# si220/Forest-SLAM

Hardware: AMD Instinct MI355X
Metric: stereo frames/sec (extract+match+local-BA) at 600p, 1/8 MI355X; ATE RMSE (higher is better)
Workload: dtype mixed: u8/u16 integer (FAST, BRIEF, Hamming, SGM), f32 (ORB angle/Harris, back-projection), f64 (PnP, BA incl. its Schur GEMM on f64 MFMA)

## Files before the change

### forest-slam_amd/csrc/fvo_internal.h

```cpp
#pragma once

#include <hip/hip_runtime.h>

#include <cmath>
#include <cstdint>
#include <string>
#include <vector>

#include "../../include/fvo.h"

#define FVO_MAX_LEVELS 12

struct OrbGeom {
  int nlevels;
  int w[FVO_MAX_LEVELS], h[FVO_MAX_LEVELS];
  float scale[FVO_MAX_LEVELS];
  int64_t off[FVO_MAX_LEVELS + 1];
  int row0[FVO_MAX_LEVELS + 1];
  int nfeat[FVO_MAX_LEVELS];
  int64_t cand_off[FVO_MAX_LEVELS + 1];
  int64_t total_px;
  int total_rows;
  int64_t cand_total;
  bool angle_pass;
};

struct ResizeTab {
  int32_t* xofs;
  int32_t* xc1;
  int32_t* yofs;
  int32_t* yc1;
  int64_t xoff[FVO_MAX_LEVELS], yoff[FVO_MAX_LEVELS];
};

constexpr int kBaMaxWindow = 21;
constexpr int kEmMaxCap = 5040;
constexpr int kRansacMaxIters = 1000;

#define FVO_KERNELS(X)                                                                                    \
  X(KN_ORB_COPY, "orb_copy_level0") X(KN_ORB_RESIZE, "orb_resize") X(KN_ORB_FAST, "orb_fast_score")       \
  X(KN_ORB_NMS_COUNT, "orb_nms_count") X(KN_ORB_ROW_SCAN, "orb_row_scan") X(KN_ORB_COMPACT, "orb_nms_compact") \
  X(KN_ORB_SELECT1, "orb_select_fast") X(KN_ORB_HARRIS, "orb_harris") X(KN_ORB_SELECT2, "orb_select_harris") \
  X(KN_ORB_OFFSETS, "orb_offsets") X(KN_ORB_ANGLE, "orb_angle") X(KN_ORB_BLUR, "orb_blur")                \
  X(KN_ORB_BRIEF, "orb_brief") X(KN_BF_ARGMIN, "bf_argmin") X(KN_BF_FINISH, "bf_finish")                  \
  X(KN_SG_VERT, "sgbm_vert") X(KN_SG_ROWS, "sgbm_rows") X(KN_SG_MEDIAN, "sgbm_median")                    \
  X(KN_BACKPROJECT, "backproject") X(KN_PNP, "pnp_ransac") X(KN_BA_STEREO, "ba_stereo")                   \
  X(KN_BA_BUILD, "ba_build") X(KN_BA_SOLVE, "ba_solve") X(KN_GATHER, "gather_matches")                    \
  X(KN_ESSENTIAL, "essential_ransac") X(KN_RECOVER, "recover_pose") X(KN_INGEST, "ingest_undistort_gray") \
  X(KN_MOTION_BLUR, "motion_blur") X(KN_MAP_XFORM, "map_transform") X(KN_VOXEL, "voxel_down_sample")      \
  X(KN_BF_KNN, "bf_knn") X(KN_BF_RATIO, "bf_ratio") X(KN_SPK_LOCAL, "speckle_local")                      \
  X(KN_SPK_SEAMS, "speckle_seams") X(KN_SPK_SUM, "speckle_sum") X(KN_SPK_APPLY, "speckle_apply")
#define FVO_KERNEL_ID(id, name) id,
enum FvoKernel { FVO_KERNELS(FVO_KERNEL_ID) KN_COUNT };
#undef FVO_KERNEL_ID

struct TimingRec {
  int id;
  hipEvent_t a, b;
};

struct fvo_ctx {
  int device = 0;
  uint64_t tmask = 0;
  std::vector<TimingRec> trecs;
  std::vector<hipEvent_t> tpool;
  fvo_config cfg{};
  OrbGeom g{};
  std::string err;
  int kp_cap = 0;
  int64_t ws_bytes = 0;
  std::vector<void*> allocs;
  uint8_t* pyr = nullptr;
  uint8_t* blur = nullptr;
  int orb_last_batch = 0;
  uint8_t* score = nullptr;
  uint32_t* cand = nullptr;
  uint64_t* hel = nullptr;
  int32_t* ncand = nullptr;
  int32_t* nsel1 = nullptr;
  int32_t* nsel2 = nullptr;
  int32_t* koff = nullptr;
  int32_t* scratch = nullptr;
  int64_t scratch_per = 0;
  ResizeTab rt{};
  int32_t* umax = nullptr;
  uint32_t* bf_rowkey = nullptr;
  uint32_t* bf_colkey = nullptr;
  uint32_t* bf_knn = nullptr;
  uint16_t* sg_V = nullptr;
  uint16_t* sg_M = nullptr;
  uint32_t* sg_ckpt = nullptr;
  int16_t* sg_raw = nullptr;
  uint64_t* sg_hand = nullptr;
  uint32_t* sg_ctl = nullptr;
  struct {
    bool valid = false;
    const void* matches = nullptr;
    const void* nmatch = nullptr;
    const void* stereo = nullptr;
    int nframes = 0, first_end = 0, nwin = 0, first_valid = 0;
  } ba_births;
  double* pnp_hyp = nullptr;
  int32_t* pnp_sub = nullptr;
  int16_t* rs_table = nullptr;
  int32_t rs_table_iters = 0;
  double* pnp_models = nullptr;
  double* pnp_ws = nullptr;
  int32_t* pnp_good = nullptr;
  void* pnp_state = nullptr;
  float* pnp_pts = nullptr;
  int32_t* pnp_plan = nullptr;
  int32_t pnp_max_iters = 0;
  uint8_t* fast_rec = nullptr;
  void* ba_ws = nullptr;
  int64_t ba_win_bytes = 0;
  hipStream_t ba_s2 = nullptr;
  hipEvent_t ba_fork = nullptr, ba_join = nullptr;
  double* em_x = nullptr;
  double* em_models = nullptr;
  int32_t* em_good = nullptr;
  int8_t* em_nmod = nullptr;
  double* em_ws = nullptr;
  void* em_state = nullptr;
  int32_t em_max_iters = 0;
  int32_t rectify_budget = FVO_RECTIFY_LDS_BYTES;
};

int fvo_fail(fvo_ctx* ctx, const std::string& msg);
#define FVO_HIP(ctx, expr)                                                                 \
  do {                                                                                     \
    hipError_t e_ = (expr);                                                                \
    if (e_ != hipSuccess) return fvo_fail(ctx, std::string(#expr) + ": " + hipGetErrorString(e_)); \
  } while (0)
#define FVO_LAUNCH_CHECK(ctx) FVO_HIP(ctx, hipGetLastError())

hipEvent_t fvo_event(fvo_ctx* ctx);
#define FVO_TIMED(ctx, id, s, ...)                               \
  do {                                                           \
    const bool t_ = ((ctx)->tmask >> (id)) & 1ull;               \
    hipEvent_t a_ = nullptr, b_ = nullptr;                       \
    if (t_) {                                                    \
      a_ = fvo_event(ctx);                                       \
      (void)hipEventRecord(a_, s);                               \
    }                                                            \
    __VA_ARGS__;                                                 \
    if (t_) {                                                    \
      b_ = fvo_event(ctx);                                       \
      (void)hipEventRecord(b_, s);                               \
      (ctx)->trecs.push_back(TimingRec{(int)(id), a_, b_});      \
    }                                                            \
  } while (0)

int orb_init(fvo_ctx* ctx);
int orb_run(fvo_ctx* ctx, const uint8_t* images, int batch, int64_t image_stride, int pitch, float* kp, uint8_t* desc,
            int32_t* counts, int cap, hipStream_t s);
int bf_init(fvo_ctx* ctx);
int bf_run(fvo_ctx* ctx, const uint8_t* q, const int32_t* nq, const uint8_t* t, const int32_t* nt, int batch, int cap,
           int32_t* matches, int32_t* nmatch, hipStream_t s);
int bf_knn_run(fvo_ctx* ctx, const uint8_t* q, const int32_t* nq, const uint8_t* t, const int32_t* nt, int batch,
               int cap, int k, int32_t* knn, hipStream_t s);
int bf_ratio_run(fvo_ctx* ctx, const uint8_t* q, const int32_t* nq, const uint8_t* t, const int32_t* nt, int batch,
                 int cap, double ratio, int mutual, int32_t* matches, int32_t* nmatch, hipStream_t s);
int sgbm_init(fvo_ctx* ctx);
int sgbm_run(fvo_ctx* ctx, const uint8_t* L, const uint8_t* R, int batch, int64_t image_stride, int pitch,
             int16_t* disp, int32_t* status, hipStream_t s);
int pose_init(fvo_ctx* ctx);
int ransac_table_init(fvo_ctx* ctx);
int orb_blur_debug(fvo_ctx* ctx);
int orb_score_debug(fvo_ctx* ctx);
int orb_retain_best_run(fvo_ctx* ctx, const float* keys, int n, int keep, int32_t* idx_out, int32_t* n_out,
                         hipStream_t s);
int backproject_run(fvo_ctx* ctx, const int16_t* disp, const float* kp0, const float* kp1, const int32_t* matches,
                    const int32_t* nmatch, int batch, int cap, const double* K, double baseline, float* P3, float* p2,
                    int32_t* npts, hipStream_t s);
int pnp_run(fvo_ctx* ctx, const float* P3, const float* p2, const int32_t* npts, int batch, int cap, const double* K,
            const double* dist, float reproj, double conf, int iters, double* rvec, double* tvec, double* T,
            int32_t* status, uint8_t* inliers, hipStream_t s);

inline bool host_inv3(const double* S, double* t) {
  double d = S[0] * (S[4] * S[8] - S[5] * S[7]) - S[1] * (S[3] * S[8] - S[5] * S[6]) + S[2] * (S[3] * S[7] - S[4] * S[6]);
  if (d == 0.) return false;
  d = 1. / d;
  t[0] = (S[4] * S[8] - S[5] * S[7]) * d;
  t[1] = (S[2] * S[7] - S[1] * S[8]) * d;
  t[2] = (S[1] * S[5] - S[2] * S[4]) * d;
  t[3] = (S[5] * S[6] - S[3] * S[8]) * d;
  t[4] = (S[0] * S[8] - S[2] * S[6]) * d;
  t[5] = (S[2] * S[3] - S[0] * S[5]) * d;
  t[6] = (S[3] * S[7] - S[4] * S[6]) * d;
  t[7] = (S[1] * S[6] - S[0] * S[7]) * d;
  t[8] = (S[0] * S[4] - S[1] * S[3]) * d;
  return true;
}
inline bool host_all_finite(const double* v, int n) {
  for (int i = 0; i < n; ++i)
    if (!std::isfinite(v[i])) return false;
  return true;
}
inline bool host_ray_w_ok(double w) { return w > 0.0 && std::isfinite(1. / w); }

inline int ingest_stripe_rows(int W, int H) {
  const int s = 4096 / (W > 1 ? W : 1);
  return s < 1 ? 1 : (s > H ? H : s);
}
int ingest_run(fvo_ctx* ctx, const uint8_t* bgr, int batch, int64_t sstride, int spitch, const double* K,
               const double* dist, uint8_t* gray, int64_t dstride, int dpitch, hipStream_t s);
int motion_blur_run(fvo_ctx* ctx, const uint8_t* img, int batch, int64_t sstride, int spitch, int ksize,
                    const int32_t* centers, const int32_t* ncent, int cap, uint8_t* mask, uint8_t* out,
                    int64_t dstride, int dpitch, hipStream_t s);
int map_transform_run(fvo_ctx* ctx, const float* pts, int stride, const int32_t* npts, int batch, int64_t cap,
                      const double* T, int32_t* count, int64_t map_cap, double* out64, float* out32, hipStream_t s);
int chain_poses_run(fvo_ctx* ctx, const double* T, const int32_t* status, const int32_t* npts, int n_seq, int n,
                    double* cum, double* cum_out, int32_t* npts_out, hipStream_t s);
struct FvoRegions {
  fvo_region r[FVO_MAX_REGIONS];
};
int copy_regions_run(fvo_ctx* ctx, int count, const fvo_region* regions, hipStream_t s);
int count_guard_run(fvo_ctx* ctx, const int32_t* cnt, const int32_t* q_cnt, int n, int sets, int32_t* status,
                    int32_t code, int32_t* nkp_out, hipStream_t s);
int64_t voxel_workspace_bytes(int64_t n);
int voxel_run(fvo_ctx* ctx, const double* pts, int64_t n, double voxel, void* ws, double* out,
              int32_t* n_out, int32_t* status, hipStream_t s);
int speckle_run(fvo_ctx* ctx, int16_t* disp, int batch, int H, int W, int64_t image_stride, int pitch, int new_val,
                int max_speckle_size, int max_diff, void* ws, hipStream_t s);
constexpr int kDenseBlock = 1024;
inline int64_t dense_frame_samples(int H, int W, int step) {
  return (int64_t)((H - 1) / step + 1) * ((W - 1) / step + 1);
}
inline int64_t dense_frame_blocks(int H, int W, int step) {
  return (dense_frame_samples(H, W, step) + kDenseBlock - 1) / kDenseBlock;
}
int dense_append_run(fvo_ctx* ctx, const int16_t* disp, int batch, int H, int W, int64_t image_stride, int pitch,
                     const double* K, double baseline, int step, int min_disp16, float z_min, float z_max,
                     const int32_t* frame_keep, const double* T, int32_t* count, int64_t map_cap, double* out64,
                     float* out32, int32_t* n_added, void* ws, hipStream_t s);
int reproject_run(fvo_ctx* ctx, const void* disp, int is_f32, int batch, int H, int W, int64_t image_stride,
                  int pitch, const double* Q, int handle_missing, uint32_t* min_key, float* out, hipStream_t s);
struct RectifyLens {
  double ir[9];
  double fx, fy, u0, v0;
  double k1, k2, p1, p2, k3, k4, k5, k6;
  int rational;
};
int rectify_map_run(fvo_ctx* ctx, const RectifyLens& L, int16_t* map1, uint16_t* map2, hipStream_t s);
int remap_run(fvo_ctx* ctx, const uint8_t* src, int batch, int64_t sstride, int spitch, int channels,
              const int16_t* map1, const uint16_t* map2, uint8_t* dst, int64_t dstride, int dpitch, hipStream_t s);
int rectify_gray_run(fvo_ctx* ctx, const uint8_t* src, int batch, int64_t sstride, int spitch, int channels,
                     const RectifyLens& L, uint8_t* gray, int64_t dstride, int dpitch, hipStream_t s);
constexpr int kSparseMaxLevels = 32;
constexpr int kSparseMaxHalfWindow = 7, kSparseMaxHalfSlide = 8;
struct SparseLevels {
  float scale[kSparseMaxLevels];
  int n;
};
int sparse_stereo_run(fvo_ctx* ctx, const uint8_t* left, const uint8_t* right, int batch, int64_t image_stride,
                      int pitch, const float* kpL, const int32_t* nL, const uint8_t* descL, const float* kpR,
                      const int32_t* nR, const uint8_t* descR, int cap, const fvo_sparse_stereo_params& p,
                      const SparseLevels& levels, const double* K, double baseline, void* ws, float* stereo,
                      int32_t* info, hipStream_t s);
int backproject_stereo_run(fvo_ctx* ctx, const float* stereo, const float* kp1, const int32_t* matches,
// ... 57 lines not shown
```

### forest-slam_amd/csrc/pose.hip

```cpp
#include <cfloat>
#include <cstdlib>
#include <type_traits>

#include "fvo_device.h"
#include "ransac.h"

namespace {

constexpr int kChunk = 64;

constexpr int kBackprojectThreads = 256;

__global__ __launch_bounds__(kBackprojectThreads) void k_backproject(
    const int16_t* __restrict__ disp, const float* __restrict__ kp0, const float* __restrict__ kp1,
    const int32_t* __restrict__ matches, const int32_t* __restrict__ nmatch, int W, int H, int cap, StereoCamF K,
    float* __restrict__ P3, float* __restrict__ p2, int32_t* __restrict__ npts) {
  const int b = blockIdx.x;
  int n = nmatch[b];
  n = n < 0 ? 0 : (n > cap ? cap : n);
  __shared__ int s_w[16];
  __shared__ int s_carry;
  if (threadIdx.x == 0) s_carry = 0;
  __syncthreads();
  for (int base = 0; base < n; base += kBackprojectThreads) {
// ... 1036 lines not shown
  for (int i = lane; i < n; i += 64) {
    const int j = i;
    dundistort(K, (double)p2[2 * j], (double)p2[2 * j + 1], &mn[2 * i]);
    acc[0] += (double)P3[3 * j];
    acc[1] += (double)P3[3 * j + 1];
    acc[2] += (double)P3[3 * j + 2];
  }
#pragma unroll
  for (int k = 0; k < 3; ++k) acc[k] = wave_sum(acc[k]);
  double Mc[3] = {acc[0] / n, acc[1] / n, acc[2] / n};
  double MM[9] = {0, 0, 0, 0, 0, 0, 0, 0, 0};
  for (int i = lane; i < n; i += 64) {
    const int j = i;
    double d[3] = {(double)P3[3 * j] - Mc[0], (double)P3[3 * j + 1] - Mc[1], (double)P3[3 * j + 2] - Mc[2]};
#pragma unroll
    for (int a = 0; a < 3; ++a)
#pragma unroll
      for (int b = 0; b < 3; ++b) MM[a * 3 + b] += d[a] * d[b];
  }
#pragma unroll
  for (int k = 0; k < 9; ++k) MM[k] = wave_sum(MM[k]);
  double W3[3], U3[9], V3[9];
  dsvd<3, 3>(MM, W3, U3, V3);
  const bool planar = W3[2] / W3[1] < 1e-3;
  if (!planar && n < 6) {
    if (lane == 0) sh.flag = 0;
    __syncthreads();
    return;
  }
  double LLp[78];
#pragma unroll
  for (int k = 0; k < 78; ++k) LLp[k] = 0;
  double Rt[9], T[3];
  if (!planar) {
    for (int i = lane; i < n; i += 64) {
      const int j = i;
      double x = -mn[2 * i], y = -mn[2 * i + 1];
      double P[3] = {(double)P3[3 * j], (double)P3[3 * j + 1], (double)P3[3 * j + 2]};
      double r0[12] = {P[0], P[1], P[2], 1., 0, 0, 0, 0, x * P[0], x * P[1], x * P[2], x};
      double r1[12] = {0, 0, 0, 0, P[0], P[1], P[2], 1., y * P[0], y * P[1], y * P[2], y};
      int k = 0;
#pragma unroll
      for (int a = 0; a < 12; ++a)
#pragma unroll
        for (int b = a; b < 12; ++b) LLp[k++] += r0[a] * r0[b] + r1[a] * r1[b];
    }
  } else {
#pragma unroll
    for (int i = 0; i < 3; ++i)
#pragma unroll
      for (int j = 0; j < 3; ++j) Rt[i * 3 + j] = V3[j * 3 + i];
    if (Rt[2] * Rt[2] + Rt[5] * Rt[5] < 1e-10)
#pragma unroll
      for (int i = 0; i < 9; ++i) Rt[i] = (i % 4 == 0);
    if (ddet3(Rt) < 0)
#pragma unroll
      for (int i = 0; i < 9; ++i) Rt[i] = -Rt[i];
#pragma unroll
    for (int i = 0; i < 3; ++i) T[i] = -(Rt[i * 3] * Mc[0] + Rt[i * 3 + 1] * Mc[1] + Rt[i * 3 + 2] * Mc[2]);
    if (lane == 0) {
#pragma unroll
      for (int i = 0; i < 9; ++i) sh.rt[i] = Rt[i];
#pragma unroll
      for (int i = 0; i < 3; ++i) sh.t3[i] = T[i];
    }
    for (int i = lane; i < n; i += 64) {
      const int j = i;
      double s0 = P3[3 * j], s1 = P3[3 * j + 1], s2 = P3[3 * j + 2];
      double X = Rt[0] * s0 + Rt[1] * s1 + Rt[2] * s2 + T[0];
      double Y = Rt[3] * s0 + Rt[4] * s1 + Rt[5] * s2 + T[1];
      double u = mn[2 * i], v = mn[2 * i + 1];
      double r0[9] = {X, Y, 1, 0, 0, 0, -u * X, -u * Y, -u};
      double r1[9] = {0, 0, 0, X, Y, 1, -v * X, -v * Y, -v};
      int k = 0;
#pragma unroll
      for (int a = 0; a < 9; ++a)
#pragma unroll
        for (int b = a; b < 9; ++b) LLp[k++] += r0[a] * r0[b] + r1[a] * r1[b];
    }
  }
#pragma unroll
  for (int k = 0; k < 78; ++k) {
    const double t = wave_sum(LLp[k]);
    if (lane == 0) sh.llp[k] = t;
  }
  __syncthreads();
  if (!planar) dlt12_null(sh.llp, sh.dlt[1], sh.dlt[2], sh.rrt);
  if (lane == 0) dlt_pose(sh, planar);
  __syncthreads();
  double prev[6];
  double lambdaLg10 = -3, prevErrNorm = DBL_MAX;
  int iters = 0;
  for (;;) {
    double e0 = lm_eval(sh, K, P3, p2, n, true);
#pragma unroll
    for (int i = 0; i < 6; ++i) prev[i] = sh.param[i];
    if (lane == 0) {
#pragma unroll
      for (int i = 0; i < 6; ++i) sh.prev[i] = prev[i];
    }
    __syncthreads();
    if (lane == 0) lm_step(sh, lambdaLg10);
    __syncthreads();
    if (iters == 0) prevErrNorm = e0;
    double errNorm;
    for (;;) {
      errNorm = lm_eval(sh, K, P3, p2, n, false);
      if (errNorm > prevErrNorm && ++lambdaLg10 <= 16) {
        if (lane == 0) lm_step(sh, lambdaLg10);
        __syncthreads();
        continue;
      }
      break;
    }
    lambdaLg10 = fmax(lambdaLg10 - 1, -16.0);
    double dn = 0, pn = 0;
#pragma unroll
    for (int i = 0; i < 6; ++i) {
      dn += (sh.param[i] - prev[i]) * (sh.param[i] - prev[i]);
      pn += prev[i] * prev[i];
    }
    double rel = sqrt(dn) / (sqrt(pn) + DBL_EPSILON);
    if (++iters >= 20 || rel < FLT_EPSILON) break;
    prevErrNorm = errNorm;
  }
  if (lane == 0) sh.flag = 1;
  __syncthreads();
}

struct PnpState {
  int maxGood, niters, best_it, n;
};

__global__ void k_pnp_table(int cap, int maxIters, int16_t* __restrict__ table) {
  const int n = blockIdx.x * blockDim.x + threadIdx.x;
  if (n < 6 || n > cap) return;
  fvo_rs::draw_subsets(n, maxIters, table + (int64_t)n * maxIters * 5);
}

__global__ void k_pnp_subsets(const int32_t* __restrict__ npts, int batch, int cap, int maxIters,
                              PnpState* __restrict__ state) {
  const int b = blockIdx.x * blockDim.x + threadIdx.x;
  if (b >= batch) return;
  int n = npts[b];
  n = n < 0 ? 0 : (n > cap ? cap : n);
  PnpState st;
  st.maxGood = 0;
  st.niters = maxIters;
  st.best_it = -1;
  st.n = n;
  state[b] = st;
}

constexpr int PNP_WS = 256;
constexpr int PW_NV = 0, PW_CWS = 48, PW_AL = 60, PW_PWS = 80, PW_US = 95, PW_MTM = 112;

constexpr int PNP_FIRST = 128;
constexpr int PNP_CS = 64, PNP_CA = 8, PNP_CB = 16;

__global__ __launch_bounds__(64) void k_pnp_plan(int batch, int maxIters, const PnpState* __restrict__ state,
                                                 int32_t* __restrict__ plan) {
  const int lane = threadIdx.x;
  int carry[3] = {0, 0, 0};
  const int C[3] = {PNP_CS, PNP_CA, PNP_CB};
  for (int b0 = 0; b0 < batch; b0 += 64) {
    const int b = b0 + lane;
    int rem = 0;
    if (b < batch) {
      const PnpState st = state[b];
      if (st.n >= 6) rem = max(0, min(st.niters, maxIters) - PNP_FIRST);
    }
#pragma unroll
    for (int k = 0; k < 3; ++k) {
      int v = (rem + C[k] - 1) / C[k];
#pragma unroll
      for (int o = 1; o < 64; o <<= 1) {
        const int y = __shfl_up(v, o, 64);
        if (lane >= o) v += y;
      }
      const int incl = v, excl = incl - (rem + C[k] - 1) / C[k];
      if (b < batch) plan[k * (batch + 1) + b] = carry[k] + excl;
      carry[k] += __shfl(incl, 63, 64);
    }
  }
  if (lane < 3) plan[lane * (batch + 1) + batch] = carry[lane];
}

__device__ __forceinline__ void pnp_unit(const int32_t* __restrict__ pre, int batch, int u, int C, int& b, int& base) {
  int lo = 0, hi = batch - 1;
  while (lo < hi) {
    const int mid = (lo + hi + 1) >> 1;
    if (pre[mid] <= u) lo = mid; else hi = mid - 1;
  }
  b = lo;
  base = PNP_FIRST + (u - pre[lo]) * C;
}

template <int C, typename Body>
__device__ __forceinline__ void pnp_units(const int32_t* __restrict__ plan, int k, int batch, int maxIters,
                                          const PnpState* __restrict__ state, Body body) {
  const int32_t* pre = plan ? plan + k * (batch + 1) : nullptr;
  const int total = plan ? pre[batch] : (int)blockIdx.x + 1;
  for (int u = blockIdx.x; u < total; u += gridDim.x) {
    int b, base, lim;
    if (plan) {
      pnp_unit(pre, batch, u, C, b, base);
      lim = maxIters;
    } else {
      b = blockIdx.y;
      base = u * C;
      lim = PNP_FIRST;
    }
    const PnpState st = state[b];
    const int hi = min(min(st.niters, maxIters), lim);
    if (st.n < 6 || base >= hi) continue;
    body(b, base, hi, st.n);
  }
}

__global__ __launch_bounds__(64, 4) void k_pnp_setup(const float* __restrict__ P3all, const float* __restrict__ p2all,
                                                  int cap, Cam K, int maxIters, int batch,
                                                  const int32_t* __restrict__ plan,
                                                  const int16_t* __restrict__ table, int table_iters,
                                                  const PnpState* __restrict__ state, double* __restrict__ ws) {
  extern __shared__ __attribute__((aligned(16))) double smt[];
  double* mt = smt + threadIdx.x;
  pnp_units<PNP_CS>(plan, 0, batch, maxIters, state, [&](int b, int base, int hi, int n) {
    const int it = base + threadIdx.x;
    if (it >= hi) return;
    const float* __restrict__ P3 = P3all + (int64_t)b * cap * 3;
    const float* __restrict__ p2 = p2all + (int64_t)b * cap * 2;
    double* w = ws + ((int64_t)b * maxIters + it) * PNP_WS;
    const int16_t* sb = table + ((int64_t)n * table_iters + it) * 5;
    EPnPd<5> e;
    e.fu = K.fx; e.fv = K.fy; e.uc = K.cx; e.vc = K.cy;
#pragma unroll
    for (int i = 0; i < 5; ++i) {
      int j = sb[i];
#pragma unroll
      for (int c = 0; c < 3; ++c) e.pws[3 * i + c] = (double)P3[j * 3 + c];
      double xy[2];
      dundistort(K, (double)p2[j * 2], (double)p2[j * 2 + 1], xy);
      float fx = (float)xy[0], fy = (float)xy[1];
      e.us[2 * i] = fx * K.fx + K.cx;
      e.us[2 * i + 1] = fy * K.fy + K.cy;
    }
    e.build_mtm<64>(mt);
#pragma unroll 8
    for (int k = 0; k < 144; ++k) w[PW_MTM + k] = mt[k * 64];
#pragma unroll
    for (int r = 0; r < 4; ++r)
#pragma unroll
      for (int k = 0; k < 3; ++k) w[PW_CWS + r * 3 + k] = e.cws[r][k];
#pragma unroll
    for (int k = 0; k < 20; ++k) w[PW_AL + k] = e.alphas[k];
#pragma unroll
    for (int k = 0; k < 15; ++k) w[PW_PWS + k] = e.pws[k];
#pragma unroll
    for (int k = 0; k < 10; ++k) w[PW_US + k] = e.us[k];
  });
}

__global__ __launch_bounds__(64) void k_pnp_hyp_a(int maxIters, int batch, const int32_t* __restrict__ plan,
                                                  const PnpState* __restrict__ state, double* __restrict__ ws) {
  __shared__ double su[8][144];
  const int g = threadIdx.x >> 3, l = threadIdx.x & 7;
  double* u = su[g];
  pnp_units<PNP_CA>(plan, 1, batch, maxIters, state, [&](int b, int base, int hi, int) {
    const int it = base + g;
    if (it >= hi) return;
    double* w = ws + ((int64_t)b * maxIters + it) * PNP_WS;
    for (int k = l; k < 144; k += 8) u[k] = w[PW_MTM + k];
    __builtin_amdgcn_s_waitcnt(0);
    __builtin_amdgcn_wave_barrier();
    jacobi12_null4_group(u, l, w + PW_NV);
  });
}

__global__ __launch_bounds__(64, 3) void k_pnp_hyp_b(const float* __restrict__ P3all, const float* __restrict__ p2all,
                                                  int cap, Cam K, float thr2, int maxIters, int batch,
                                                  const int32_t* __restrict__ plan,
                                                  const PnpState* __restrict__ state, const double* __restrict__ ws,
                                                  double* __restrict__ model, int32_t* __restrict__ good) {
  __shared__ double sL[16][66];
  const int g = threadIdx.x >> 2, l = threadIdx.x & 3;
  double* L = sL[g];
  pnp_units<PNP_CB>(plan, 2, batch, maxIters, state, [&](int b, int base, int hi, int n) {
    const int it = base + g;
    if (it >= hi) return;
    const float* __restrict__ P3 = P3all + (int64_t)b * cap * 3;
    const float* __restrict__ p2 = p2all + (int64_t)b * cap * 2;
    const double* w = ws + ((int64_t)b * maxIters + it) * PNP_WS;
    EPnPd<5, true> e;
    e.fu = K.fx; e.fv = K.fy; e.uc = K.cx; e.vc = K.cy;
    e.pws = w + PW_PWS;
    e.us = w + PW_US;
    e.alphas = w + PW_AL;
    e.cws = reinterpret_cast<const double (*)[3]>(w + PW_CWS);
    const double (*nv)[12] = reinterpret_cast<const double (*)[12]>(w + PW_NV);
    if (l == 0) e.prep(nv, L, L + 60);
    __builtin_amdgcn_s_waitcnt(0);
    __builtin_amdgcn_wave_barrier();
    double R[9], t[3];
    const double err = e.approx(l < 3 ? l + 1 : 3, L, L + 60, nv, R, t);
    const int gb = threadIdx.x & ~3;
    const double e1 = __shfl(err, gb + 1, 64), e2 = __shfl(err, gb + 2, 64);
    int sel = 0;
    double best = __shfl(err, gb, 64);
    if (e1 < best) { best = e1; sel = 1; }
    if (e2 < best) sel = 2;
#pragma unroll
    for (int k = 0; k < 9; ++k) R[k] = __shfl(R[k], gb + sel, 64);
#pragma unroll
    for (int k = 0; k < 3; ++k) t[k] = __shfl(t[k], gb + sel, 64);
    double r[3], dR[27];
    rod_R2r(R, r);
    if (l == 0) {
      double* mo = model + ((int64_t)b * maxIters + it) * 6;
      for (int i = 0; i < 3; ++i) { mo[i] = r[i]; mo[3 + i] = t[i]; }
    }
    rod_r2R(r, R, dR);
    int gcount = 0;
#pragma nounroll
    for (int i = l; i < n; i += 4) {
      double M[3] = {(double)P3[3 * i], (double)P3[3 * i + 1], (double)P3[3 * i + 2]}, uv[2];
      dproject(K, R, dR, t, M, uv, nullptr);
      float du = p2[2 * i] - (float)uv[0], dv = p2[2 * i + 1] - (float)uv[1];
      gcount += (du * du + dv * dv) <= thr2;
    }
    gcount += __shfl_xor(gcount, 1, 4);
    gcount += __shfl_xor(gcount, 2, 4);
    if (l == 0) good[(int64_t)b * maxIters + it] = gcount;
  });
}

__global__ __launch_bounds__(64) void k_pnp_replay(int maxIters, int it_lo, int it_hi, double conf,
                                                   const int32_t* __restrict__ good, PnpState* __restrict__ state) {
  const int b = blockIdx.x, lane = threadIdx.x;
  PnpState st = state[b];
  if (st.n < 6) return;
  for (int base = it_lo; base < it_hi && base < st.niters; base += 64) {
    const int it = base + lane;
    const int g = (it < it_hi && it < st.niters) ? good[(int64_t)b * maxIters + it] : 0;
    for (int j = 0; j < 64; ++j) {
      if (base + j >= it_hi || base + j >= st.niters) break;
      const int gj = __builtin_amdgcn_readlane(g, j);
      if (gj > max(st.maxGood, 4)) {
        st.best_it = base + j;
        st.maxGood = gj;
        st.niters = update_num_iters(conf, (double)(st.n - gj) / st.n, 5, st.niters);
      }
    }
  }
  if (lane == 0) state[b] = st;
}

__global__ __launch_bounds__(64, 2) void k_pnp_refine(const float* __restrict__ P3all, const float* __restrict__ p2all,
                                                   int cap, Cam K, float thr2, int maxIters,
                                                   const PnpState* __restrict__ state,
                                                   const double* __restrict__ model, double* __restrict__ rvec,
                                                   double* __restrict__ tvec, double* __restrict__ T,
                                                   int32_t* __restrict__ status, uint8_t* __restrict__ inliers,
                                                   int32_t* __restrict__ inl_idx, double* __restrict__ mn_buf,
                                                   float* __restrict__ pts) {
  __shared__ PnpShared sh;
  __shared__ float s_pts[5 * kRefineLds];
  const int b = blockIdx.x, lane = threadIdx.x;
  const PnpState st = state[b];
  const int n = st.n;
  const float* P3 = P3all + (int64_t)b * cap * 3;
  const float* p2 = p2all + (int64_t)b * cap * 2;
  double* Tout = T + (int64_t)b * 16;
  if (n < 6 || st.maxGood <= 0) {
    if (lane < 16) Tout[lane] = (lane % 5 == 0) ? 1.0 : 0.0;
    if (lane < 3) { rvec[b * 3 + lane] = 0; tvec[b * 3 + lane] = 0; }
    if (inliers)
      for (int i = lane; i < cap; i += 64) inliers[(int64_t)b * cap + i] = 0;
    if (lane == 0) status[b] = n < 6 ? -1 : 0;
    return;
  }
  const double* mo = model + ((int64_t)b * maxIters + st.best_it) * 6;
  if (lane < 6) sh.best[lane] = mo[lane];
  __syncthreads();
  int* inl = inl_idx + (int64_t)b * cap;
  {
    double r[3] = {sh.best[0], sh.best[1], sh.best[2]}, t[3] = {sh.best[3], sh.best[4], sh.best[5]};
    double R[9], dR[27];
    rod_r2R(r, R, dR);
    int carry = 0;
    for (int base = 0; base < n; base += 64) {
      int i = base + lane;
      bool f = false;
      if (i < n) {
        double M[3] = {(double)P3[3 * i], (double)P3[3 * i + 1], (double)P3[3 * i + 2]}, uv[2];
        dproject(K, R, dR, t, M, uv, nullptr);
        float du = p2[2 * i] - (float)uv[0], dv = p2[2 * i + 1] - (float)uv[1];
        f = du * du + dv * dv <= thr2;
        if (inliers) inliers[(int64_t)b * cap + i] = (uint8_t)f;
      }
      unsigned long long m = __ballot(f);
      if (f) {
        const int k = carry + __popcll(m & ((1ull << lane) - 1ull));
        inl[k] = i;
        if (k < kRefineLds) {
          s_pts[3 * k] = P3[3 * i];
          s_pts[3 * k + 1] = P3[3 * i + 1];
          s_pts[3 * k + 2] = P3[3 * i + 2];
          s_pts[3 * kRefineLds + 2 * k] = p2[2 * i];
          s_pts[3 * kRefineLds + 2 * k + 1] = p2[2 * i + 1];
        }
      }
      carry += __popcll(m);
    }
    if (inliers)
      for (int i = n + lane; i < cap; i += 64) inliers[(int64_t)b * cap + i] = 0;
    if (lane == 0) sh.ninl = carry;
  }
  __syncthreads();
  const int ninl = sh.ninl;
  const float* Pc = s_pts;
  const float* Qc = s_pts + 3 * kRefineLds;
  if (ninl > kRefineLds) {
    float* gP = pts + (int64_t)b * cap * 5;
    float* gQ = gP + 3 * cap;
    for (int k = lane; k < ninl; k += 64) {
      const int i = inl[k];
      gP[3 * k] = P3[3 * i];
      gP[3 * k + 1] = P3[3 * i + 1];
      gP[3 * k + 2] = P3[3 * i + 2];
      gQ[2 * k] = p2[2 * i];
      gQ[2 * k + 1] = p2[2 * i + 1];
    }
    __syncthreads();
    Pc = gP;
    Qc = gQ;
  }
  lm_refine(sh, K, Pc, Qc, ninl, mn_buf + (int64_t)b * cap * 2);
  double out[6];
  for (int i = 0; i < 6; ++i) out[i] = sh.flag ? sh.param[i] : sh.best[i];
  if (lane == 0) {
    double R[9];
    rod_r2R(out, R, nullptr);
    for (int i = 0; i < 3; ++i) {
      rvec[b * 3 + i] = out[i];
      tvec[b * 3 + i] = out[3 + i];
      Tout[i * 4 + 0] = R[i * 3];
      Tout[i * 4 + 1] = R[i * 3 + 1];
      Tout[i * 4 + 2] = R[i * 3 + 2];
      Tout[i * 4 + 3] = out[3 + i];
    }
    Tout[12] = 0; Tout[13] = 0; Tout[14] = 0; Tout[15] = 1;
    status[b] = 1;
  }
}

}

int pose_init(fvo_ctx* ctx) {
  ctx->pnp_max_iters = kRansacMaxIters;
  const int64_t B = ctx->cfg.max_batch, n = B * ctx->kp_cap, it = B * ctx->pnp_max_iters;
  int rc;
  if ((rc = fvo_alloc(ctx, &ctx->pnp_sub, n)) || (rc = fvo_alloc(ctx, &ctx->pnp_hyp, 2 * n)) ||
      (rc = ransac_table_init(ctx)) || (rc = fvo_alloc(ctx, &ctx->pnp_models, it * 6)) ||
      (rc = fvo_alloc(ctx, &ctx->pnp_ws, it * PNP_WS)) ||
      (rc = hipFuncSetAttribute((const void*)k_pnp_setup, hipFuncAttributeMaxDynamicSharedMemorySize,
                                144 * 64 * (int)sizeof(double)) == hipSuccess ? 0 : fvo_fail(ctx, "pnp: LDS attribute")) ||
      (rc = fvo_alloc(ctx, &ctx->pnp_good, it)) || (rc = fvo_alloc(ctx, (PnpState**)&ctx->pnp_state, B)) ||
      (rc = fvo_alloc(ctx, &ctx->pnp_plan, 3 * (B + 1))) || (rc = fvo_alloc(ctx, &ctx->pnp_pts, 5 * n)))
    return rc;
  return 0;
}

int ransac_table_init(fvo_ctx* ctx) {
  if (ctx->rs_table) return 0;
  ctx->rs_table_iters = kRansacMaxIters;
  int rc;
  if ((rc = fvo_alloc(ctx, &ctx->rs_table, (int64_t)(ctx->kp_cap + 1) * ctx->rs_table_iters * 5))) return rc;
  hipLaunchKernelGGL(k_pnp_table, dim3((ctx->kp_cap + 1 + 63) / 64), dim3(64), 0, 0, ctx->kp_cap,
                     ctx->rs_table_iters, ctx->rs_table);
  FVO_LAUNCH_CHECK(ctx);
  FVO_HIP(ctx, hipDeviceSynchronize());
  return 0;
}

int backproject_run(fvo_ctx* ctx, const int16_t* disp, const float* kp0, const float* kp1, const int32_t* matches,
                    const int32_t* nmatch, int batch, int cap, const double* K, double baseline, float* P3, float* p2,
                    int32_t* npts, hipStream_t s) {
  FVO_TIMED(ctx, KN_BACKPROJECT, s,
            hipLaunchKernelGGL(k_backproject, dim3(batch), dim3(kBackprojectThreads), 0, s, disp, kp0, kp1, matches,
                               nmatch, ctx->cfg.width, ctx->cfg.height, cap, stereo_cam(K, baseline), P3, p2, npts));
  FVO_LAUNCH_CHECK(ctx);
  return 0;
}

int pnp_run(fvo_ctx* ctx, const float* P3, const float* p2, const int32_t* npts, int batch, int cap, const double* K,
            const double* dist, float reproj, double conf, int iters, double* rvec, double* tvec, double* T,
            int32_t* status, uint8_t* inliers, hipStream_t s) {
  Cam c{K[0], K[4], K[2], K[5], {dist[0], dist[1], dist[2], dist[3], dist[4]}};
  const float thr2 = (float)((double)reproj * reproj);
  const int maxIters = iters;
  PnpState* st = (PnpState*)ctx->pnp_state;
  const int first = std::min(maxIters, PNP_FIRST);
  auto hyp = [&](const int32_t* plan, dim3 gs, dim3 ga, dim3 gb, int lo, int hi) {
    hipLaunchKernelGGL(k_pnp_setup, gs, dim3(64), 144 * 64 * sizeof(double), s, P3, p2, cap, c, maxIters, batch, plan,
                       ctx->rs_table, ctx->rs_table_iters, st, ctx->pnp_ws);
    hipLaunchKernelGGL(k_pnp_hyp_a, ga, dim3(64), 0, s, maxIters, batch, plan, st, ctx->pnp_ws);
    hipLaunchKernelGGL(k_pnp_hyp_b, gb, dim3(64), 0, s, P3, p2, cap, c, thr2, maxIters, batch, plan, st, ctx->pnp_ws,
                       ctx->pnp_models, ctx->pnp_good);
    hipLaunchKernelGGL(k_pnp_replay, dim3(batch), dim3(64), 0, s, maxIters, lo, hi, conf, ctx->pnp_good, st);
  };
  FVO_TIMED(ctx, KN_PNP, s, {
    hipLaunchKernelGGL(k_pnp_subsets, dim3((batch + 63) / 64), dim3(64), 0, s, npts, batch, cap, maxIters, st);
    hyp(nullptr, dim3((first + PNP_CS - 1) / PNP_CS, batch), dim3((first + PNP_CA - 1) / PNP_CA, batch),
        dim3((first + PNP_CB - 1) / PNP_CB, batch), 0, first);
    if (maxIters > first) {
      hipLaunchKernelGGL(k_pnp_plan, dim3(1), dim3(64), 0, s, batch, maxIters, st, ctx->pnp_plan);
      const int gs = batch * ((PNP_FIRST + PNP_CS - 1) / PNP_CS), ga = batch * ((PNP_FIRST + PNP_CA - 1) / PNP_CA),
                gb = batch * ((PNP_FIRST + PNP_CB - 1) / PNP_CB);
      hyp(ctx->pnp_plan, dim3(gs), dim3(ga), dim3(gb), first, maxIters);
    }
    hipLaunchKernelGGL(k_pnp_refine, dim3(batch), dim3(64), 0, s, P3, p2, cap, c, thr2, maxIters, st,
                       ctx->pnp_models, rvec, tvec, T, status, inliers, ctx->pnp_sub, ctx->pnp_hyp, ctx->pnp_pts);
  });
  FVO_LAUNCH_CHECK(ctx);
  return 0;
}
```

Before: 6095.

## Fuse PnP RANSAC setup, null-space and model kernels into one LDS-resident kernel

Merges the three PnP hypothesis kernels (EPnP setup, Jacobi null-space, model/inlier scoring) into a single kernel where each 8-lane group keeps its per-hypothesis workspace in LDS instead of a global 256-double scratch buffer. The M^T M build is now spread across 8 lanes rather than one thread per hypothesis, and the scan plan shrinks to a single unit size. This removes global-memory round trips for the workspace and two kernel launches per RANSAC stage. In exchange, control-point and barycentric computation is serialized on lane 0, inlier counting uses 8 lanes instead of 4, and the larger static LDS block may limit occupancy.

```diff
diff --git a/forest-slam_amd/csrc/fvo_internal.h b/forest-slam_amd/csrc/fvo_internal.h
--- a/forest-slam_amd/csrc/fvo_internal.h
+++ b/forest-slam_amd/csrc/fvo_internal.h
@@ -105,7 +105,6 @@
   int16_t* rs_table = nullptr;
   int32_t rs_table_iters = 0;
   double* pnp_models = nullptr;
-  double* pnp_ws = nullptr;
   int32_t* pnp_good = nullptr;
   void* pnp_state = nullptr;
   float* pnp_pts = nullptr;
diff --git a/forest-slam_amd/csrc/pose.hip b/forest-slam_amd/csrc/pose.hip
--- a/forest-slam_amd/csrc/pose.hip
+++ b/forest-slam_amd/csrc/pose.hip
@@ -1212,17 +1212,28 @@
   state[b] = st;
 }
 
-constexpr int PNP_WS = 256;
-constexpr int PW_NV = 0, PW_CWS = 48, PW_AL = 60, PW_PWS = 80, PW_US = 95, PW_MTM = 112;
+constexpr int PS_CWS = 0, PS_AL = 12, PS_PWS = 32, PS_US = 47, PS_N = 57;
+
+struct PnpHypLds {
+  double u[8][144];
+  double nv[8][48];
+  double st[8][PS_N];
+};
+__shared__ PnpHypLds s_hyp;
+
+__device__ __forceinline__ void wave_lds_sync() {
+  __builtin_amdgcn_fence(__ATOMIC_RELEASE, "wavefront");
+  __builtin_amdgcn_wave_barrier();
+  __builtin_amdgcn_fence(__ATOMIC_ACQUIRE, "wavefront");
+}
 
 constexpr int PNP_FIRST = 128;
-constexpr int PNP_CS = 64, PNP_CA = 8, PNP_CB = 16;
+constexpr int PNP_C = 8;
 
 __global__ __launch_bounds__(64) void k_pnp_plan(int batch, int maxIters, const PnpState* __restrict__ state,
                                                  int32_t* __restrict__ plan) {
   const int lane = threadIdx.x;
-  int carry[3] = {0, 0, 0};
-  const int C[3] = {PNP_CS, PNP_CA, PNP_CB};
+  int carry = 0;
   for (int b0 = 0; b0 < batch; b0 += 64) {
     const int b = b0 + lane;
     int rem = 0;
@@ -1230,45 +1241,41 @@
       const PnpState st = state[b];
       if (st.n >= 6) rem = max(0, min(st.niters, maxIters) - PNP_FIRST);
     }
-#pragma unroll
-    for (int k = 0; k < 3; ++k) {
-      int v = (rem + C[k] - 1) / C[k];
-#pragma unroll
-      for (int o = 1; o < 64; o <<= 1) {
-        const int y = __shfl_up(v, o, 64);
-        if (lane >= o) v += y;
-      }
-      const int incl = v, excl = incl - (rem + C[k] - 1) / C[k];
-      if (b < batch) plan[k * (batch + 1) + b] = carry[k] + excl;
-      carry[k] += __shfl(incl, 63, 64);
-    }
-  }
-  if (lane < 3) plan[lane * (batch + 1) + batch] = carry[lane];
-}
-
-__device__ __forceinline__ void pnp_unit(const int32_t* __restrict__ pre, int batch, int u, int C, int& b, int& base) {
+    const int units = (rem + PNP_C - 1) / PNP_C;
+    int v = units;
+#pragma unroll
+    for (int o = 1; o < 64; o <<= 1) {
+      const int y = __shfl_up(v, o, 64);
+      if (lane >= o) v += y;
+    }
+    if (b < batch) plan[b] = carry + v - units;
+    carry += __shfl(v, 63, 64);
+  }
+  if (lane == 0) plan[batch] = carry;
+}
+
+__device__ __forceinline__ void pnp_unit(const int32_t* __restrict__ pre, int batch, int u, int& b, int& base) {
   int lo = 0, hi = batch - 1;
   while (lo < hi) {
     const int mid = (lo + hi + 1) >> 1;
     if (pre[mid] <= u) lo = mid; else hi = mid - 1;
   }
   b = lo;
-  base = PNP_FIRST + (u - pre[lo]) * C;
-}
-
-template <int C, typename Body>
-__device__ __forceinline__ void pnp_units(const int32_t* __restrict__ plan, int k, int batch, int maxIters,
+  base = PNP_FIRST + (u - pre[lo]) * PNP_C;
+}
+
+template <typename Body>
+__device__ __forceinline__ void pnp_units(const int32_t* __restrict__ plan, int batch, int maxIters,
                                           const PnpState* __restrict__ state, Body body) {
-  const int32_t* pre = plan ? plan + k * (batch + 1) : nullptr;
-  const int total = plan ? pre[batch] : (int)blockIdx.x + 1;
+  const int total = plan ? plan[batch] : (int)blockIdx.x + 1;
   for (int u = blockIdx.x; u < total; u += gridDim.x) {
     int b, base, lim;
     if (plan) {
-      pnp_unit(pre, batch, u, C, b, base);
+      pnp_unit(plan, batch, u, b, base);
       lim = maxIters;
     } else {
       b = blockIdx.y;
-      base = u * C;
+      base = u * PNP_C;
       lim = PNP_FIRST;
     }
     const PnpState st = state[b];
@@ -1278,119 +1285,120 @@
   }
 }
 
-__global__ __launch_bounds__(64, 4) void k_pnp_setup(const float* __restrict__ P3all, const float* __restrict__ p2all,
-                                                  int cap, Cam K, int maxIters, int batch,
-                                                  const int32_t* __restrict__ plan,
-                                                  const int16_t* __restrict__ table, int table_iters,
-                                                  const PnpState* __restrict__ state, double* __restrict__ ws) {
-  extern __shared__ __attribute__((aligned(16))) double smt[];
-  double* mt = smt + threadIdx.x;
-  pnp_units<PNP_CS>(plan, 0, batch, maxIters, state, [&](int b, int base, int hi, int n) {
-    const int it = base + threadIdx.x;
-    if (it >= hi) return;
-    const float* __restrict__ P3 = P3all + (int64_t)b * cap * 3;
-    const float* __restrict__ p2 = p2all + (int64_t)b * cap * 2;
-    double* w = ws + ((int64_t)b * maxIters + it) * PNP_WS;
-    const int16_t* sb = table + ((int64_t)n * table_iters + it) * 5;
+__device__ __attribute__((noinline)) void pnp_hyp_setup(const float* __restrict__ P3, const float* __restrict__ p2,
+                                                        const int16_t* __restrict__ sb, const Cam K, int g, int l) {
+  double* st = s_hyp.st[g];
+  if (l < 5) {
+    const int j = sb[l];
+#pragma unroll
+    for (int c = 0; c < 3; ++c) st[PS_PWS + 3 * l + c] = (double)P3[j * 3 + c];
+    double xy[2];
+    dundistort(K, (double)p2[j * 2], (double)p2[j * 2 + 1], xy);
+    const float fx = (float)xy[0], fy = (float)xy[1];
+    st[PS_US + 2 * l] = fx * K.fx + K.cx;
+    st[PS_US + 2 * l + 1] = fy * K.fy + K.cy;
+  }
+  wave_lds_sync();
+  if (l == 0) {
     EPnPd<5> e;
-    e.fu = K.fx; e.fv = K.fy; e.uc = K.cx; e.vc = K.cy;
+#pragma unroll
+    for (int k = 0; k < 15; ++k) e.pws[k] = st[PS_PWS + k];
+    e.choose_control_points();
+    e.barycentric();
+#pragma unroll
+    for (int r = 0; r < 4; ++r)
+#pragma unroll
+      for (int k = 0; k < 3; ++k) st[PS_CWS + r * 3 + k] = e.cws[r][k];
+#pragma unroll
+    for (int k = 0; k < 20; ++k) st[PS_AL + k] = e.alphas[k];
+  }
+  wave_lds_sync();
+  const double fu = K.fx, fv = K.fy, uc = K.cx, vc = K.cy;
+  double* mtm = s_hyp.u[g];
+#pragma nounroll
+  for (int k = l; k < 144; k += 8) {
+    const int a = k / 12, bb = k - a * 12;
+    const int ja = a / 3, ca = a - ja * 3, jb = bb / 3, cb = bb - jb * 3;
+    double s = 0.0;
 #pragma unroll
     for (int i = 0; i < 5; ++i) {
-      int j = sb[i];
-#pragma unroll
-      for (int c = 0; c < 3; ++c) e.pws[3 * i + c] = (double)P3[j * 3 + c];
-      double xy[2];
-      dundistort(K, (double)p2[j * 2], (double)p2[j * 2 + 1], xy);
-      float fx = (float)xy[0], fy = (float)xy[1];
-      e.us[2 * i] = fx * K.fx + K.cx;
-      e.us[2 * i + 1] = fy * K.fy + K.cy;
-    }
-    e.build_mtm<64>(mt);
-#pragma unroll 8
-    for (int k = 0; k < 144; ++k) w[PW_MTM + k] = mt[k * 64];
-#pragma unroll
-    for (int r = 0; r < 4; ++r)
-#pragma unroll
-      for (int k = 0; k < 3; ++k) w[PW_CWS + r * 3 + k] = e.cws[r][k];
-#pragma unroll
-    for (int k = 0; k < 20; ++k) w[PW_AL + k] = e.alphas[k];
-#pragma unroll
-    for (int k = 0; k < 15; ++k) w[PW_PWS + k] = e.pws[k];
-#pragma unroll
-    for (int k = 0; k < 10; ++k) w[PW_US + k] = e.us[k];
-  });
-}
-
-__global__ __launch_bounds__(64) void k_pnp_hyp_a(int maxIters, int batch, const int32_t* __restrict__ plan,
-                                                  const PnpState* __restrict__ state, double* __restrict__ ws) {
-  __shared__ double su[8][144];
+      const double aa = st[PS_AL + 4 * i + ja], ab = st[PS_AL + 4 * i + jb];
+      const double u = st[PS_US + 2 * i], v = st[PS_US + 2 * i + 1];
+      const double m1a = ca == 0 ? aa * fu : ca == 1 ? 0.0 : aa * (uc - u);
+      const double m1b = cb == 0 ? ab * fu : cb == 1 ? 0.0 : ab * (uc - u);
+      const double m2a = ca == 0 ? 0.0 : ca == 1 ? aa * fv : aa * (vc - v);
+      const double m2b = cb == 0 ? 0.0 : cb == 1 ? ab * fv : ab * (vc - v);
+      s += m1a * m1b;
+      s += m2a * m2b;
+    }
+    mtm[k] = s;
+  }
+  wave_lds_sync();
+}
+
+__device__ __attribute__((noinline)) void pnp_hyp_model(const float* __restrict__ P3, const float* __restrict__ p2,
+                                                        int n, const Cam K, float thr2, int g, int l,
+                                                        double* __restrict__ mo, int32_t* __restrict__ good) {
+  const double* st = s_hyp.st[g];
+  double* L = s_hyp.u[g];
+  EPnPd<5, true> e;
+  e.fu = K.fx; e.fv = K.fy; e.uc = K.cx; e.vc = K.cy;
+  e.pws = st + PS_PWS;
+  e.us = st + PS_US;
+  e.alphas = st + PS_AL;
+  e.cws = reinterpret_cast<const double (*)[3]>(st + PS_CWS);
+  const double (*nv)[12] = reinterpret_cast<const double (*)[12]>(s_hyp.nv[g]);
+  if (l == 0) e.prep(nv, L, L + 60);
+  wave_lds_sync();
+  double R[9], t[3];
+  const double err = e.approx(l < 3 ? l + 1 : 3, L, L + 60, nv, R, t);
+  const int gb = threadIdx.x & ~7;
+  const double e1 = __shfl(err, gb + 1, 64), e2 = __shfl(err, gb + 2, 64);
+  int sel = 0;
+  double best = __shfl(err, gb, 64);
+  if (e1 < best) { best = e1; sel = 1; }
+  if (e2 < best) sel = 2;
+#pragma unroll
+  for (int k = 0; k < 9; ++k) R[k] = __shfl(R[k], gb + sel, 64);
+#pragma unroll
+  for (int k = 0; k < 3; ++k) t[k] = __shfl(t[k], gb + sel, 64);
+  double r[3], dR[27];
+  rod_R2r(R, r);
+  if (l == 0) {
+    for (int i = 0; i < 3; ++i) { mo[i] = r[i]; mo[3 + i] = t[i]; }
+  }
+  rod_r2R(r, R, dR);
+  int gcount = 0;
+#pragma nounroll
+  for (int i = l; i < n; i += 8) {
+    double M[3] = {(double)P3[3 * i], (double)P3[3 * i + 1], (double)P3[3 * i + 2]}, uv[2];
+    dproject(K, R, dR, t, M, uv, nullptr);
+    float du = p2[2 * i] - (float)uv[0], dv = p2[2 * i + 1] - (float)uv[1];
+    gcount += (du * du + dv * dv) <= thr2;
+  }
+  gcount += __shfl_xor(gcount, 1, 8);
+  gcount += __shfl_xor(gcount, 2, 8);
+  gcount += __shfl_xor(gcount, 4, 8);
+  if (l == 0) *good = gcount;
+  wave_lds_sync();
+}
+
+__global__ __launch_bounds__(64, 3) void k_pnp_hyp(const float* __restrict__ P3all, const float* __restrict__ p2all,
+                                                int cap, Cam K, float thr2, int maxIters, int batch,
+                                                const int32_t* __restrict__ plan, const int16_t* __restrict__ table,
+                                                int table_iters, const PnpState* __restrict__ state,
+                                                double* __restrict__ model, int32_t* __restrict__ good) {
   const int g = threadIdx.x >> 3, l = threadIdx.x & 7;
-  double* u = su[g];
-  pnp_units<PNP_CA>(plan, 1, batch, maxIters, state, [&](int b, int base, int hi, int) {
-    const int it = base + g;
-    if (it >= hi) return;
-    double* w = ws + ((int64_t)b * maxIters + it) * PNP_WS;
-    for (int k = l; k < 144; k += 8) u[k] = w[PW_MTM + k];
-    __builtin_amdgcn_s_waitcnt(0);
-    __builtin_amdgcn_wave_barrier();
-    jacobi12_null4_group(u, l, w + PW_NV);
-  });
-}
-
-__global__ __launch_bounds__(64, 3) void k_pnp_hyp_b(const float* __restrict__ P3all, const float* __restrict__ p2all,
-                                                  int cap, Cam K, float thr2, int maxIters, int batch,
-                                                  const int32_t* __restrict__ plan,
-                                                  const PnpState* __restrict__ state, const double* __restrict__ ws,
-                                                  double* __restrict__ model, int32_t* __restrict__ good) {
-  __shared__ double sL[16][66];
-  const int g = threadIdx.x >> 2, l = threadIdx.x & 3;
-  double* L = sL[g];
-  pnp_units<PNP_CB>(plan, 2, batch, maxIters, state, [&](int b, int base, int hi, int n) {
+  pnp_units(plan, batch, maxIters, state, [&](int b, int base, int hi, int n) {
     const int it = base + g;
     if (it >= hi) return;
     const float* __restrict__ P3 = P3all + (int64_t)b * cap * 3;
     const float* __restrict__ p2 = p2all + (int64_t)b * cap * 2;
-    const double* w = ws + ((int64_t)b * maxIters + it) * PNP_WS;
-    EPnPd<5, true> e;
-    e.fu = K.fx; e.fv = K.fy; e.uc = K.cx; e.vc = K.cy;
-    e.pws = w + PW_PWS;
-    e.us = w + PW_US;
-    e.alphas = w + PW_AL;
-    e.cws = reinterpret_cast<const double (*)[3]>(w + PW_CWS);
-    const double (*nv)[12] = reinterpret_cast<const double (*)[12]>(w + PW_NV);
-    if (l == 0) e.prep(nv, L, L + 60);
-    __builtin_amdgcn_s_waitcnt(0);
-    __builtin_amdgcn_wave_barrier();
-    double R[9], t[3];
-    const double err = e.approx(l < 3 ? l + 1 : 3, L, L + 60, nv, R, t);
-    const int gb = threadIdx.x & ~3;
-    const double e1 = __shfl(err, gb + 1, 64), e2 = __shfl(err, gb + 2, 64);
-    int sel = 0;
-    double best = __shfl(err, gb, 64);
-    if (e1 < best) { best = e1; sel = 1; }
-    if (e2 < best) sel = 2;
-#pragma unroll
-    for (int k = 0; k < 9; ++k) R[k] = __shfl(R[k], gb + sel, 64);
-#pragma unroll
-    for (int k = 0; k < 3; ++k) t[k] = __shfl(t[k], gb + sel, 64);
-    double r[3], dR[27];
-    rod_R2r(R, r);
-    if (l == 0) {
-      double* mo = model + ((int64_t)b * maxIters + it) * 6;
-      for (int i = 0; i < 3; ++i) { mo[i] = r[i]; mo[3 + i] = t[i]; }
-    }
-    rod_r2R(r, R, dR);
-    int gcount = 0;
-#pragma nounroll
-    for (int i = l; i < n; i += 4) {
-      double M[3] = {(double)P3[3 * i], (double)P3[3 * i + 1], (double)P3[3 * i + 2]}, uv[2];
-      dproject(K, R, dR, t, M, uv, nullptr);
-      float du = p2[2 * i] - (float)uv[0], dv = p2[2 * i + 1] - (float)uv[1];
-      gcount += (du * du + dv * dv) <= thr2;
-    }
-    gcount += __shfl_xor(gcount, 1, 4);
-    gcount += __shfl_xor(gcount, 2, 4);
-    if (l == 0) good[(int64_t)b * maxIters + it] = gcount;
+    pnp_hyp_setup(P3, p2, table + ((int64_t)n * table_iters + it) * 5, K, g, l);
+    jacobi12_null4_group(s_hyp.u[g], l, s_hyp.nv[g]);
+    wave_lds_sync();
+    pnp_hyp_model(P3, p2, n, K, thr2, g, l, model + ((int64_t)b * maxIters + it) * 6,
+                  good + (int64_t)b * maxIters + it);
   });
 }
 
@@ -1522,11 +1530,8 @@
   int rc;
   if ((rc = fvo_alloc(ctx, &ctx->pnp_sub, n)) || (rc = fvo_alloc(ctx, &ctx->pnp_hyp, 2 * n)) ||
       (rc = ransac_table_init(ctx)) || (rc = fvo_alloc(ctx, &ctx->pnp_models, it * 6)) ||
-      (rc = fvo_alloc(ctx, &ctx->pnp_ws, it * PNP_WS)) ||
-      (rc = hipFuncSetAttribute((const void*)k_pnp_setup, hipFuncAttributeMaxDynamicSharedMemorySize,
-                                144 * 64 * (int)sizeof(double)) == hipSuccess ? 0 : fvo_fail(ctx, "pnp: LDS attribute")) ||
       (rc = fvo_alloc(ctx, &ctx->pnp_good, it)) || (rc = fvo_alloc(ctx, (PnpState**)&ctx->pnp_state, B)) ||
-      (rc = fvo_alloc(ctx, &ctx->pnp_plan, 3 * (B + 1))) || (rc = fvo_alloc(ctx, &ctx->pnp_pts, 5 * n)))
+      (rc = fvo_alloc(ctx, &ctx->pnp_plan, B + 1)) || (rc = fvo_alloc(ctx, &ctx->pnp_pts, 5 * n)))
     return rc;
   return 0;
 }
@@ -1561,23 +1566,17 @@
   const int maxIters = iters;
   PnpState* st = (PnpState*)ctx->pnp_state;
   const int first = std::min(maxIters, PNP_FIRST);
-  auto hyp = [&](const int32_t* plan, dim3 gs, dim3 ga, dim3 gb, int lo, int hi) {
-    hipLaunchKernelGGL(k_pnp_setup, gs, dim3(64), 144 * 64 * sizeof(double), s, P3, p2, cap, c, maxIters, batch, plan,
-                       ctx->rs_table, ctx->rs_table_iters, st, ctx->pnp_ws);
-    hipLaunchKernelGGL(k_pnp_hyp_a, ga, dim3(64), 0, s, maxIters, batch, plan, st, ctx->pnp_ws);
-    hipLaunchKernelGGL(k_pnp_hyp_b, gb, dim3(64), 0, s, P3, p2, cap, c, thr2, maxIters, batch, plan, st, ctx->pnp_ws,
-                       ctx->pnp_models, ctx->pnp_good);
+  auto hyp = [&](const int32_t* plan, dim3 grid, int lo, int hi) {
+    hipLaunchKernelGGL(k_pnp_hyp, grid, dim3(64), 0, s, P3, p2, cap, c, thr2, maxIters, batch, plan, ctx->rs_table,
+                       ctx->rs_table_iters, st, ctx->pnp_models, ctx->pnp_good);
     hipLaunchKernelGGL(k_pnp_replay, dim3(batch), dim3(64), 0, s, maxIters, lo, hi, conf, ctx->pnp_good, st);
   };
   FVO_TIMED(ctx, KN_PNP, s, {
     hipLaunchKernelGGL(k_pnp_subsets, dim3((batch + 63) / 64), dim3(64), 0, s, npts, batch, cap, maxIters, st);
-    hyp(nullptr, dim3((first + PNP_CS - 1) / PNP_CS, batch), dim3((first + PNP_CA - 1) / PNP_CA, batch),
-        dim3((first + PNP_CB - 1) / PNP_CB, batch), 0, first);
+    hyp(nullptr, dim3((first + PNP_C - 1) / PNP_C, batch), 0, first);
     if (maxIters > first) {
       hipLaunchKernelGGL(k_pnp_plan, dim3(1), dim3(64), 0, s, batch, maxIters, st, ctx->pnp_plan);
-      const int gs = batch * ((PNP_FIRST + PNP_CS - 1) / PNP_CS), ga = batch * ((PNP_FIRST + PNP_CA - 1) / PNP_CA),
-                gb = batch * ((PNP_FIRST + PNP_CB - 1) / PNP_CB);
-      hyp(ctx->pnp_plan, dim3(gs), dim3(ga), dim3(gb), first, maxIters);
+      hyp(ctx->pnp_plan, dim3(batch * (PNP_FIRST / PNP_C)), first, maxIters);
     }
     hipLaunchKernelGGL(k_pnp_refine, dim3(batch), dim3(64), 0, s, P3, p2, cap, c, thr2, maxIters, st,
                        ctx->pnp_models, rvec, tvec, T, status, inliers, ctx->pnp_sub, ctx->pnp_hyp, ctx->pnp_pts);
```

Result: no change. 6092 (-0.1%).
